# jackyko1991/vnet-tensorflow

Measured on AMD Instinct MI355X. Metric: training patches/sec (128^3x1ch fp32), higher is better.
Workload: dtype f32

## Files before the change

vnet_tensorflow_amd/csrc/conv_x3.h:

```cpp
#pragma once
#include "conv_kernels.h"

namespace {

constexpr int X3_TZ = 2, X3_TY = 8, X3_TX = 16;
constexpr int X3_IZ = X3_TZ + 4, X3_IY = X3_TY + 4, X3_IX = X3_TX + 4;
constexpr int X3_NV = X3_IZ * X3_IY * X3_IX;

template <bool W8>
struct X3G {
    static constexpr int TZ = W8 ? 4 : 2;
    static constexpr int IZ = TZ + 4, IY = X3_IY, IX = W8 ? 12 : X3_IX;
    static constexpr int ROWB = IX * 16;
    static constexpr int ZB = IY * ROWB + (W8 ? 64 : 0);
    static constexpr int PLANEB = IZ * ZB;
    static constexpr int PIECEB = 2 * PLANEB;
    static constexpr int TILEB = 3 * PIECEB;
    static constexpr int LDS = TILEB + 2 * 8 * 32 * 4;
    static constexpr int SPER = W8 ? 8 : 12;
};
static_assert(X3G<false>::PLANEB == X3_NV * 16 && X3G<false>::PLANEB % 256 == 0 && X3G<true>::PLANEB % 256 == 0, "tile planes");
static_assert((2 * X3G<true>::ZB) % 256 == 128, "lanes 8..15 of the narrow brick: the other half of the 256-byte bank row");
constexpr int X3_LDS = X3G<false>::LDS;

template <int K, int N, typename F>
__device__ __forceinline__ void x3_for_impl(F&& f) {
    if constexpr (K < N) { f(std::integral_constant<int, K>{}); x3_for_impl<K + 1, N>(f); }
}
template <int N, typename F>
__device__ __forceinline__ void x3_for(F&& f) { x3_for_impl<0, N>(f); }

typedef const __attribute__((address_space(1))) u32x4* x3_gw_t;
template <int NP>
__device__ __forceinline__ void x3_load_a(bf16x8 (&A)[NP][3], const u32x4* __restrict__ wbase, unsigned u0, unsigned ustride, int lane) {
    x3_for<NP * 3>([&](auto I) {
        constexpr int p = decltype(I)::value / 3, s = decltype(I)::value % 3;
        A[p][s] = __builtin_bit_cast(bf16x8, *(x3_gw_t)(wbase + (u0 + (unsigned)p * ustride + (unsigned)s * 64u) + lane));
    });
}
__device__ __forceinline__ void x3_load_a1(bf16x8 (&A)[3], const u32x4* __restrict__ wbase, unsigned u0, int lane) {
    x3_for<3>([&](auto I) {
        constexpr int s = decltype(I)::value;
        A[s] = __builtin_bit_cast(bf16x8, *(x3_gw_t)(wbase + (u0 + (unsigned)s * 64u) + lane));
    });
}

template <typename G>
__device__ __forceinline__ void x3_read_b(bf16x8 (&B)[3], const unsigned char* p) {
    B[0] = *reinterpret_cast<const bf16x8*>(p);
    B[1] = *reinterpret_cast<const bf16x8*>(p + G::PIECEB);
    B[2] = *reinterpret_cast<const bf16x8*>(p + 2 * G::PIECEB);
}

#define X3_PROD_A(k) ((k) == 0 ? 2 : (k) == 1 ? 0 : (k) == 2 ? 1 : (k) == 3 ? 1 : (k) == 4 ? 0 : 0)
#define X3_PROD_B(k) ((k) == 0 ? 0 : (k) == 1 ? 2 : (k) == 2 ? 1 : (k) == 3 ? 0 : (k) == 4 ? 1 : 0)

template <typename G, int DY0, int NDY, int A0 = 0, int NA = NDY>
__device__ __forceinline__ void x3_zrows(f32x4 (&acc)[8], const unsigned char* bz, const bf16x8 (&A)[NA][3]) {
    constexpr int J0 = DY0, J1 = DY0 + NDY + 7;
    bf16x8 Bn[3];
    x3_read_b<G>(Bn, bz + J0 * G::ROWB);
    x3_for<J1 - J0>([&](auto JI) {
        constexpr int jr = J0 + decltype(JI)::value;
        bf16x8 B[3] = {Bn[0], Bn[1], Bn[2]};
        if constexpr (jr + 1 < J1) x3_read_b<G>(Bn, bz + (jr + 1) * G::ROWB);
        __builtin_amdgcn_sched_barrier(0);
        x3_for<6 * NDY>([&](auto KI) {
            constexpr int k = decltype(KI)::value / NDY, d = decltype(KI)::value % NDY, m = jr - DY0 - d;
            if constexpr (m >= 0 && m < 8)
                acc[m] = __builtin_amdgcn_mfma_f32_16x16x32_bf16(A[A0 + d][X3_PROD_A(k)], B[X3_PROD_B(k)], acc[m], 0, 0, 0);
        });
        __builtin_amdgcn_sched_barrier(0);
    });
}

template <typename G, int A0, int NA>
__device__ __forceinline__ void x3_yrows_pairs(f32x4 (&acc)[8], const unsigned char* by, const bf16x8 (&A)[NA][3]) {
    bf16x8 Bn[3];
    x3_read_b<G>(Bn, by);
    x3_for<10>([&](auto KI) {
        constexpr int k = decltype(KI)::value;
        bf16x8 B[3] = {Bn[0], Bn[1], Bn[2]};
        if constexpr (k + 1 < 10) x3_read_b<G>(Bn, by + (k + 1) * G::ROWB);
        __builtin_amdgcn_sched_barrier(0);
        x3_for<6>([&](auto TI) {
            constexpr int t = decltype(TI)::value;
            if constexpr (k < 8) acc[k] = __builtin_amdgcn_mfma_f32_16x16x32_bf16(A[A0][X3_PROD_A(t)], B[X3_PROD_B(t)], acc[k], 0, 0, 0);
            if constexpr (k >= 2) acc[k - 2] = __builtin_amdgcn_mfma_f32_16x16x32_bf16(A[A0 + 1][X3_PROD_A(t)], B[X3_PROD_B(t)], acc[k - 2], 0, 0, 0);
        });
        __builtin_amdgcn_sched_barrier(0);
    });
}
template <typename G, int A0, int NA>
__device__ __forceinline__ void x3_yrows_single(f32x4 (&acc)[8], const unsigned char* b0, const bf16x8 (&A)[NA][3]) {
    bf16x8 Bn[3];
    x3_read_b<G>(Bn, b0 + 4 * G::ROWB);
    x3_for<8>([&](auto MI) {
        constexpr int m = decltype(MI)::value;
        bf16x8 B[3] = {Bn[0], Bn[1], Bn[2]};
        if constexpr (m + 1 < 8) x3_read_b<G>(Bn, b0 + (m + 5) * G::ROWB);
        __builtin_amdgcn_sched_barrier(0);
        x3_for<6>([&](auto TI) {
            constexpr int t = decltype(TI)::value;
            acc[m] = __builtin_amdgcn_mfma_f32_16x16x32_bf16(A[A0][X3_PROD_A(t)], B[X3_PROD_B(t)], acc[m], 0, 0, 0);
        });
        __builtin_amdgcn_sched_barrier(0);
    });
}

template <bool STATS, int NB, bool W8 = false>
__global__ void __launch_bounds__(512) __attribute__((amdgpu_waves_per_eu(2, 2))) conv5_x3_kernel(ConvArgs a) {
    constexpr int NT = 512;
    using G = X3G<W8>;
    using XT = XTile<X3_IZ, X3_IY, X3_IX, NT>;
    static_assert(XT::PER * XT::RPI == XT::ROWS && XT::PER == X3G<false>::SPER, "every staging pass covers whole tile rows");
    extern __shared__ __attribute__((aligned(16))) unsigned char smem[];
    unsigned char* tile = smem;
    float* red = reinterpret_cast<float*>(smem);
    float* sred = reinterpret_cast<float*>(smem + G::TILEB);
    const int tid = threadIdx.x;
    const int lane = tid & 63, wave = __builtin_amdgcn_readfirstlane(tid >> 6);
    const int j = lane & 15, g = lane >> 4, half = g & 1, hi = g >> 1;
    const int grp = wave >> 2, kw = wave & 3;

    const int base0 = W8 ? half * G::PLANEB + (grp + 2 * (j >> 3)) * G::ZB + (j & 7) * 16
                         : half * G::PLANEB + ((grp * G::IY) * G::IX + j) * 16;
    const unsigned char* bZ = tile + base0 + hi * G::ZB;
    const unsigned char* bY = tile + base0 + hi * G::ROWB + 4 * G::ZB;
    const unsigned char* b0 = tile + base0 + 4 * G::ZB;
    const unsigned char* bX = b0 + hi * 16;

    const int ncob = a.CoutP >> 4, ncobg = ncob / NB;
    const int nbrick = a.B * a.nbz * a.nby * a.nbx;
    const int nks = a.nz;
    const int nitems = nbrick * ncobg * nks;
    const int G8 = gridDim.x >> 3;
    const int per_xcd = (nitems + 7) >> 3;
    const int xcd = blockIdx.x & 7, slot = blockIdx.x >> 3;
    const int i_lo = xcd * per_xcd, i_hi = min(nitems, i_lo + per_xcd);
    if (i_lo + slot >= i_hi) return;
    const int nmine = (i_hi - i_lo - slot + G8 - 1) / G8;
    const int nch = a.cps;
    const int nsteps = nmine * nch;
    const unsigned astride = (unsigned)ncob * 3u * 64u;
    const u32x4* wbase = reinterpret_cast<const u32x4*>(a.wp);

    auto item_coords = [&](int it, int& b, int& bz, int& by, int& bx, int& cob) {
        int item = (i_lo + slot + it * G8) / nks;
        cob = (item % ncobg) * NB; item /= ncobg;
        bx = item % a.nbx; item /= a.nbx;
        by = item % a.nby; item /= a.nby;
        bz = item % a.nbz; b = item / a.nbz;
    };
    typedef const __attribute__((address_space(1))) f32x4* gf4_t;
    f32x4 pv[G::SPER];
    const int stid = W8 ? (tid < 384 ? tid : tid - 128) : (tid < XT::RPI * XT::COLS ? tid : tid - XT::COLS);
    constexpr int SCOLS = W8 ? 32 : XT::COLS;
    const int sr0 = stid / SCOLS, scol = stid - sr0 * SCOLS;
    const int six = scol >> 2, scq = scol & 3;
    auto tile_issue = [&](int step) {
        const int it = step / nch, ch = ((i_lo + slot + it * G8) % nks) * nch + (step - it * nch);
        int b, bz, by, bx, cob;
        item_coords(it, b, bz, by, bx, cob);
        const int c0 = ch * 16;
        const bool first = c0 < a.C0;
        const int cs = first ? a.C0 : a.C1;
        const float* src = (first ? a.x0 + c0 : a.x1 + (c0 - a.C0)) + (size_t)b * a.Di * a.Hi * a.Wi * cs;
        if constexpr (W8) {
            const int gz0 = bz * G::TZ - 2, gy = by * X3_TY - 2 + sr0;
            const bool yok = (unsigned)gy < (unsigned)a.Hi;
            const int rs = a.Wi * cs;
            const int off0 = (gy * a.Wi + six) * cs + scq * 4;
            x3_for<G::SPER>([&](auto KI) {
                constexpr int k = decltype(KI)::value;
                const int gz = gz0 + k;
                const bool ok = yok && (unsigned)gz < (unsigned)a.Di;
                const int off = off0 + gz * a.Hi * rs;
                gf4_t p = ok ? (gf4_t)(src + off) : (gf4_t)(vnet_zero_line);
                pv[k] = *p;
            });
        } else {
            const int gz0 = bz * X3_TZ - 2, gy = by * X3_TY - 2 + sr0, gx = bx * X3_TX - 2 + six;
            const bool xok = (unsigned)gx < (unsigned)a.Wi;
            const bool yok0 = xok && (unsigned)gy < (unsigned)a.Hi, yok1 = xok && (unsigned)(gy + 6) < (unsigned)a.Hi;
            const int rs = a.Wi * cs;
            const int off0 = (gy * a.Wi + gx) * cs + scq * 4;
            x3_for<XT::PER>([&](auto KI) {
                constexpr int k = decltype(KI)::value;
                const int gz = gz0 + (k >> 1);
                const bool ok = ((k & 1) ? yok1 : yok0) && (unsigned)gz < (unsigned)a.Di;
                const int off = off0 + gz * a.Hi * rs + (k & 1) * 6 * rs;
                gf4_t p = ok ? (gf4_t)(src + off) : (gf4_t)(vnet_zero_line);
                pv[k] = *p;
            });
        }
    };
    const unsigned cbase = (unsigned)((scq >> 1) * G::PLANEB + (six + (W8 ? 2 : 0)) * 16 + (scq & 1) * 8 + sr0 * G::ROWB);
    auto tile_commit = [&](const unsigned sgn) {
        unsigned cb = cbase;
        asm volatile("" : "+v"(cb));
        unsigned char* base = tile + cb;
        x3_for<G::SPER>([&](auto KI) {
            constexpr int k = decltype(KI)::value;
            u32x2 h, m, l;
            x3_split4(make_float4(__uint_as_float(__float_as_uint(pv[k][0]) ^ sgn), __uint_as_float(__float_as_uint(pv[k][1]) ^ sgn),
                                  __uint_as_float(__float_as_uint(pv[k][2]) ^ sgn), __uint_as_float(__float_as_uint(pv[k][3]) ^ sgn)), h, m, l);
            unsigned char* dst = base + k * (W8 ? G::ZB : XT::RPI * G::ROWB);
            *reinterpret_cast<u32x2*>(dst) = h;
            *reinterpret_cast<u32x2*>(dst + G::PIECEB) = m;
            *reinterpret_cast<u32x2*>(dst + 2 * G::PIECEB) = l;
        });
    };
    auto zero_halo = [&]() {
        if constexpr (W8) {
            int t0 = tid;
            asm volatile("" : "+v"(t0));
#pragma unroll 1
            for (int q = t0; q < 3 * 2 * 96 * 4; q += NT) {
                const int c = q & 3, row = (q >> 2) % 96, ph = q / (96 * 4);
                const int iz = row / 12, iy = row - iz * 12;
                *reinterpret_cast<u32x4*>(tile + ph * G::PLANEB + iz * G::ZB + iy * G::ROWB + (c < 2 ? c : c + 8) * 16) = u32x4{0u, 0u, 0u, 0u};
            }
        }
    };
    zero_halo();
    tile_issue(0);
    tile_commit(0u);
    __syncthreads();

    f32x4 acc[NB][8];
    VNET_STAMP_DECL;
    for (int step = 0; step < nsteps; ++step) {
        VNET_STAMP_STEP(step);
        VNET_STAMP(0);
        const int it = step / nch, lc = step - it * nch, ks = (i_lo + slot + it * G8) % nks, ch = ks * nch + lc;
        const bool first = lc == 0, last = lc == nch - 1, more = step + 1 < nsteps;
        int b, bz, by, bx, cob;
        item_coords(it, b, bz, by, bx, cob);
        if (first) x3_for<8 * NB>([&](auto MI) { acc[decltype(MI)::value / 8][decltype(MI)::value % 8] = f32x4{0.f, 0.f, 0.f, 0.f}; });
        else x3_for<8 * NB>([&](auto MI) { acc[decltype(MI)::value / 8][decltype(MI)::value % 8] = -acc[decltype(MI)::value / 8][decltype(MI)::value % 8]; });
        const int kc = (kw + ch) & 3;
        x3_for<NB>([&](auto NBI) {
            constexpr int nb = decltype(NBI)::value;
            const unsigned wc = (unsigned)(ch * X3_NPAIR * ncob + cob + nb) * 3u * 64u;
            bf16x8 A[5][3];
            if (grp) __builtin_amdgcn_s_setprio(1); else __builtin_amdgcn_s_setprio(0);
            x3_load_a<5>(A, wbase, wc + (unsigned)(kc * 5) * astride, astride, lane);
            __builtin_amdgcn_sched_barrier(0);
            x3_zrows<G, 0, 5>(acc[nb], bZ + kc * 16, A);
            __builtin_amdgcn_sched_barrier(0);
            if constexpr (nb == 0) VNET_STAMP(1);
            x3_load_a<5>(A, wbase, wc + (unsigned)(25 + kc * 5) * astride, astride, lane);
            __builtin_amdgcn_sched_barrier(0);
            x3_zrows<G, 0, 5>(acc[nb], bZ + 2 * G::ZB + kc * 16, A);
            __builtin_amdgcn_sched_barrier(0);
            if constexpr (nb == 0) VNET_STAMP(2);
            x3_load_a1(A[0], wbase, wc + (unsigned)(50 + kc * 2) * astride, lane);
            x3_load_a1(A[1], wbase, wc + (unsigned)(51 + kc * 2) * astride, lane);
            x3_load_a1(A[2], wbase, wc + (unsigned)(60 + (kc & 1)) * astride, lane);
            x3_load_a1(A[3], wbase, wc + 62u * astride, lane);
            __builtin_amdgcn_sched_barrier(0);
            if (grp) __builtin_amdgcn_s_setprio(0); else __builtin_amdgcn_s_setprio(1);
            if constexpr (nb == NB - 1) tile_issue(min(step + 1, nsteps - 1));
            __builtin_amdgcn_sched_barrier(0);
            x3_yrows_pairs<G, 0, 5>(acc[nb], bY + kc * 16, A);
            if (kc < 2) x3_yrows_single<G, 2, 5>(acc[nb], bX + kc * 32, A);
            if (kc == 3) x3_yrows_single<G, 3, 5>(acc[nb], b0 + 4 * 16, A);
            __builtin_amdgcn_sched_barrier(0);
            if constexpr (nb == 0) VNET_STAMP(3);
            {
                const int p0 = kc == 0 ? 20 : kc == 1 ? 23 : kc == 2 ? 46 : 49;
                const int p1 = kc == 0 ? 21 : kc == 1 ? 24 : kc == 2 ? 47 : 58;
                const int p2 = kc == 0 ? 22 : kc == 1 ? 45 : kc == 2 ? 48 : 59;
                x3_load_a1(A[0], wbase, wc + (unsigned)p0 * astride, lane);
                x3_load_a1(A[1], wbase, wc + (unsigned)p1 * astride, lane);
                x3_load_a1(A[2], wbase, wc + (unsigned)p2 * astride, lane);
            }
            __builtin_amdgcn_sched_barrier(0);
            if (kc == 0) {
                x3_zrows<G, 0, 3, 0, 5>(acc[nb], bZ + 4 * 16, A);
            } else if (kc == 1) {
                x3_zrows<G, 3, 2, 0, 5>(acc[nb], bZ + 4 * 16, A);
                x3_zrows<G, 0, 1, 2, 5>(acc[nb], bZ + 2 * G::ZB + 4 * 16, A);
            } else if (kc == 2) {
                x3_zrows<G, 1, 3, 0, 5>(acc[nb], bZ + 2 * G::ZB + 4 * 16, A);
            } else {
                x3_zrows<G, 4, 1, 0, 5>(acc[nb], bZ + 2 * G::ZB + 4 * 16, A);
                x3_yrows_pairs<G, 1, 5>(acc[nb], bY + 4 * 16, A);
            }
            __builtin_amdgcn_sched_barrier(0);
        });
        VNET_STAMP(4);
        __builtin_amdgcn_s_setprio(0);
        __syncthreads();
        VNET_STAMP(5);
        if (last) {
            const bool flip = lc & 1;
            x3_for<8 * NB>([&](auto MI) {
                constexpr int nb = decltype(MI)::value / 8, m = decltype(MI)::value % 8;
                *reinterpret_cast<f32x4*>(red + (((wave * NB + nb) * 8 + m) * 64 + lane) * 4) = flip ? -acc[nb][m] : acc[nb][m];
            });
            __syncthreads();
            x3_for<NB>([&](auto NBI) {
            constexpr int nb = decltype(NBI)::value;
            const int co0 = (cob + nb) * 16, co = co0 + 4 * g;
            f32x4 o[2];
            x3_for<2>([&](auto TI) {
                constexpr int t = decltype(TI)::value;
                const int m = 2 * kw + t;
                constexpr int WS = NB * 8 * 64 * 4;
                const float* rp = red + (((grp * 4 * NB + nb) * 8 + m) * 64 + lane) * 4;
                o[t] = (*reinterpret_cast<const f32x4*>(rp) + *reinterpret_cast<const f32x4*>(rp + WS)) +
                       (*reinterpret_cast<const f32x4*>(rp + 2 * WS) + *reinterpret_cast<const f32x4*>(rp + 3 * WS));
            });
            float bias4[4] = {0.f, 0.f, 0.f, 0.f};
            if (a.bias && co < a.Cout) {
                const float4 bb = *reinterpret_cast<const float4*>(a.bias + co);
                bias4[0] = bb.x; bias4[1] = bb.y; bias4[2] = bb.z; bias4[3] = bb.w;
            }
            float s1[4] = {0.f, 0.f, 0.f, 0.f}, s2[4] = {0.f, 0.f, 0.f, 0.f};
            const int oz = W8 ? bz * G::TZ + grp + 2 * (j >> 3) : bz * X3_TZ + grp, ox = W8 ? (j & 7) : bx * X3_TX + j;
            x3_for<2>([&](auto TI) {
                constexpr int t = decltype(TI)::value;
                const int oy = by * X3_TY + 2 * kw + t;
                if (oz < a.Do && oy < a.Ho && ox < a.Wo && co < a.Cout) {
                    const size_t ov = ((size_t)(b * a.Do + oz) * a.Ho + oy) * a.Wo + ox;
                    if (a.part) {
                        *reinterpret_cast<f32x4*>(a.part + (size_t)ks * a.part_stride + ov * a.CoutP + co) = o[t];
                        return;
                    }
                    float e[4] = {o[t][0] + bias4[0], o[t][1] + bias4[1], o[t][2] + bias4[2], o[t][3] + bias4[3]};
                    if constexpr (STATS) {
                        float4 rr = make_float4(0.f, 0.f, 0.f, 0.f);
                        if (a.res) rr = *reinterpret_cast<const float4*>(a.res + ov * a.Cout + co);
                        const float vv[4] = {e[0] + rr.x, e[1] + rr.y, e[2] + rr.z, e[3] + rr.w};
                        s1[0] += vv[0]; s1[1] += vv[1]; s1[2] += vv[2]; s1[3] += vv[3];
                        s2[0] += vv[0] * vv[0]; s2[1] += vv[1] * vv[1]; s2[2] += vv[2] * vv[2]; s2[3] += vv[3] * vv[3];
                    }
                    float* p = (co < a.Cy0) ? a.y0 + ov * a.Cy0 + co : a.y1 + ov * a.Cy1 + (co - a.Cy0);
                    if (a.accum) {
                        const float4 old = *reinterpret_cast<const float4*>(a.accsrc ? a.accsrc + ov * a.Cy0 + co : p);
                        e[0] += old.x; e[1] += old.y; e[2] += old.z; e[3] += old.w;
                    }
                    *reinterpret_cast<float4*>(p) = make_float4(e[0], e[1], e[2], e[3]);
                }
            });
            if constexpr (STATS) {
                x3_for<4>([&](auto KI) {
                    constexpr int k = decltype(KI)::value;
                    s1[k] = row16_sum(s1[k]); s2[k] = row16_sum(s2[k]);
                    if (j == 0) { sred[(nb * 8 + wave) * 32 + 4 * g + k] = s1[k]; sred[(nb * 8 + wave) * 32 + 16 + 4 * g + k] = s2[k]; }
                });
            }
            });
            __syncthreads();
            if constexpr (STATS) {
                int brick = (i_lo + slot + it * G8) / (ncobg * nks);
                x3_for<NB>([&](auto NBI) {
                    constexpr int nb = decltype(NBI)::value;
                    stats_row_write<8, 16>(sred + nb * 8 * 32, a.stats, (size_t)brick, (cob + nb) * 16, a.Cout, tid);
                });
            }
        }
        VNET_STAMP(6);
        if (last) zero_halo();
        if (more) tile_commit(((last ? 0 : lc + 1) & 1) ? 0x80000000u : 0u);
        VNET_STAMP(7);
        __syncthreads();
        VNET_STAMP(8);
        VNET_STAMP_FLUSH(step, wave, lane, 9);
    }
}

template <bool W8>
struct XWG {
    static constexpr int TZ = W8 ? 4 : 2;
    static constexpr int IZ = TZ + 4, IX = W8 ? 12 : X3_IX;
    static constexpr int XROW = IX * 32, XPLANE = X3_IY * XROW;
    static constexpr int XPB = IZ * XPLANE;
    static constexpr int DPB = 2 * X3_TY * 16 * 32;
    static constexpr int LDS = 3 * XPB + 3 * DPB;
    static constexpr int XHALF = W8 ? 2 * XPLANE : 8 * 32;
    static constexpr int XPER = W8 ? 8 : 12;
};
static_assert(XWG<false>::XROW % 256 == 128 && XWG<true>::XROW % 256 == 128, "row pairs of a k-step on disjoint banks");
constexpr int XW_LDS = XWG<false>::LDS;

__device__ __forceinline__ void xw_frag(bf16x8 (&F)[3], const unsigned char* lo, const unsigned char* hi, int pieceb) {
    typedef s16x4 __attribute__((address_space(3))) * lp;
#pragma unroll
    for (int s = 0; s < 3; ++s) {
        const s16x4 a = __builtin_amdgcn_ds_read_tr16_b64_v4i16((lp)(lo + s * pieceb));
        const s16x4 b = __builtin_amdgcn_ds_read_tr16_b64_v4i16((lp)(hi + s * pieceb));
        const s16x8 v = {a[0], a[1], a[2], a[3], b[0], b[1], b[2], b[3]};
        F[s] = __builtin_bit_cast(bf16x8, v);
    }
}

__device__ __forceinline__ void xw_mfma6(f32x4& acc, const bf16x8 (&A)[3], const bf16x8 (&B)[3]) {
#pragma unroll
    for (int k = 0; k < 6; ++k) acc = __builtin_amdgcn_mfma_f32_16x16x32_bf16(A[X3_PROD_A(k)], B[X3_PROD_B(k)], acc, 0, 0, 0);
}

template <bool W8>
__global__ void __launch_bounds__(512) __attribute__((amdgpu_waves_per_eu(2, 2))) wgrad5_x3_kernel(WgradArgs a) {
    constexpr int NT = 512;
    using G = XWG<W8>;
    constexpr int XW_XPB = G::XPB, XW_DPB = G::DPB, XW_XROW = G::XROW, XW_XPLANE = G::XPLANE;
    using XT = XTile<X3_IZ, X3_IY, X3_IX, NT>;
    static_assert(XT::PER == XWG<false>::XPER, "staging passes of the wide brick");
    extern __shared__ __attribute__((aligned(16))) unsigned char smem[];
    unsigned char* xt = smem;
    unsigned char* dyt = smem + 3 * XW_XPB;
    const int tid = threadIdx.x;
    const int lane = tid & 63, wave = __builtin_amdgcn_readfirstlane(tid >> 6);
    const int i = lane & 15, g = lane >> 4;
    const int split = blockIdx.x;
    const int chunk = blockIdx.y / a.ncob, cob = blockIdx.y - chunk * a.ncob;
    const int co0 = cob * 16;

    const int lane_x = W8 ? ((g & 1) * G::IX + (i >> 2)) * 32 + (g >> 1) * G::XHALF + (i & 3) * 8
                            : (((g & 1) * X3_IX + (g >> 1) * 8) + (i >> 2)) * 32 + (i & 3) * 8;
    const unsigned char* pb[3];
#pragma unroll
    for (int c = 0; c < 3; ++c) {
        const int q = 3 * wave + c, dz = q / 5, dx = q - dz * 5;
        pb[c] = xt + dz * XW_XPLANE + dx * 32 + lane_x;
    }
    const bool extra = wave < 5;
    const unsigned char* pe = xt + 4 * XW_XPLANE + (extra ? wave : 0) * XW_XROW + 4 * 32 + lane_x;
    const int lane_d = (((g & 1) * 16 + (g >> 1) * 8) + (i >> 2)) * 32 + (i & 3) * 8;
    const unsigned char* pa_lo = dyt + lane_d + (g & 1) * 128;
    const unsigned char* pa_hi = dyt + lane_d + (1 - (g & 1)) * 128;

    f32x4 acc[16];
#pragma unroll
    for (int t = 0; t < 16; ++t) acc[t] = f32x4{0.f, 0.f, 0.f, 0.f};

    float4 px[G::XPER], pd[2];
    auto brick_coords = [&](int brick, int& b, int& bz, int& by, int& bx) {
        bx = brick % a.nbx; brick /= a.nbx;
        by = brick % a.nby; brick /= a.nby;
        bz = brick % a.nbz; b = brick / a.nbz;
    };
    auto issue = [&](int brick) {
        int b, bz, by, bx;
        brick_coords(brick, b, bz, by, bx);
        if constexpr (W8) {
            const int stid = tid < 384 ? tid : tid - 128;
            const int iy = stid >> 5, col = stid & 31;
            const int c = chunk * 16 + (col & 3) * 4;
            const bool first = c < a.C0;
            const int cs = first ? a.C0 : a.C1;
            const float* src = (first ? a.x0 + c : a.x1 + (c - a.C0)) + (size_t)b * a.Di * a.Hi * a.Wi * cs;
            const int gz0 = bz * G::TZ - 2, gy = by * X3_TY - 2 + iy;
            const bool yok = (unsigned)gy < (unsigned)a.Hi;
            const int rs = a.Wi * cs, off0 = (gy * a.Wi + (col >> 2)) * cs;
#pragma unroll
            for (int k = 0; k < G::XPER; ++k) {
                const int gz = gz0 + k;
                const bool ok = yok && (unsigned)gz < (unsigned)a.Di;
                const float4 t = *reinterpret_cast<const float4*>(src + (ok ? off0 + gz * a.Hi * rs : 0));
                px[k] = ok ? t : make_float4(0.f, 0.f, 0.f, 0.f);
            }
        } else {
            XT::template issue_part<0, XT::PER>(px, a.x0, a.x1, a.C0, a.C1, chunk, b, bz * X3_TZ - 2, by * X3_TY - 2, bx * X3_TX - 2, a.Di, a.Hi, a.Wi, tid);
        }
#pragma unroll
        for (int k = 0; k < 2; ++k) {
            const int q = tid + k * NT;
            const int v = q >> 2, cq = q & 3;
            const int vx = v & 15, vy = (v >> 4) & 7, vz = v >> 7;
            const int oz = W8 ? bz * G::TZ + vz + 2 * (vx >> 3) : bz * X3_TZ + vz, oy = by * X3_TY + vy, ox = W8 ? (vx & 7) : bx * X3_TX + vx;
            const int c = co0 + cq * 4;
            const bool ok = oz < a.Do && oy < a.Ho && ox < a.Wo && c < a.Cout;
            const size_t ov = ok ? ((size_t)(b * a.Do + oz) * a.Ho + oy) * a.Wo + ox : 0;
            const float4 t = *reinterpret_cast<const float4*>(a.dy + ov * a.Cout + (ok ? c : 0));
            pd[k] = ok ? t : make_float4(0.f, 0.f, 0.f, 0.f);
        }
    };
    auto commit = [&](const bool neg) {
        if constexpr (W8) {
            const int stid = tid < 384 ? tid : tid - 128;
            unsigned char* base = xt + (stid >> 5) * XW_XROW + (((stid & 31) >> 2) + 2) * 32 + (stid & 3) * 8;
#pragma unroll
            for (int k = 0; k < G::XPER; ++k) {
                u32x2 h, m, l;
                x3_split4(px[k], h, m, l);
                unsigned char* dst = base + k * XW_XPLANE;
                *reinterpret_cast<u32x2*>(dst) = h;
                *reinterpret_cast<u32x2*>(dst + XW_XPB) = m;
                *reinterpret_cast<u32x2*>(dst + 2 * XW_XPB) = l;
            }
        } else {
        const int r0 = tid / XT::COLS, col = tid - r0 * XT::COLS;
        if (r0 < XT::RPI) {
            unsigned char* base = xt + (col >> 2) * 32 + (col & 3) * 8;
#pragma unroll
            for (int k = 0; k < XT::PER; ++k) {
                const int row = r0 + k * XT::RPI;
                u32x2 h, m, l;
                x3_split4(px[k], h, m, l);
                unsigned char* dst = base + row * XW_XROW;
                *reinterpret_cast<u32x2*>(dst) = h;
                *reinterpret_cast<u32x2*>(dst + XW_XPB) = m;
                *reinterpret_cast<u32x2*>(dst + 2 * XW_XPB) = l;
            }
        }
        }
#pragma unroll
        for (int k = 0; k < 2; ++k) {
            const int q = tid + k * NT;
            const int v = q >> 2, cq = q & 3;
            const int vx = v & 15, row = v >> 4;
            u32x2 h, m, l;
            const float4 dv = neg ? make_float4(-pd[k].x, -pd[k].y, -pd[k].z, -pd[k].w) : pd[k];
            x3_split4(dv, h, m, l);
            unsigned char* dst = dyt + (row * 16 + (vx ^ ((row & 1) << 2))) * 32 + cq * 8;
            *reinterpret_cast<u32x2*>(dst) = h;
            *reinterpret_cast<u32x2*>(dst + XW_DPB) = m;
            *reinterpret_cast<u32x2*>(dst + 2 * XW_DPB) = l;
        }
    };

    bool neg = false;
    if constexpr (W8) {
        for (int q = tid; q < 3 * G::IZ * X3_IY * 4 * 2; q += NT) {
            const int hf = q & 1, c = (q >> 1) & 3, row = (q >> 3) % (G::IZ * X3_IY), piece = q / (8 * G::IZ * X3_IY);
            *reinterpret_cast<u32x4*>(xt + piece * XW_XPB + row * XW_XROW + (c < 2 ? c : c + 8) * 32 + hf * 16) = u32x4{0u, 0u, 0u, 0u};
        }
    }
    if (split < a.nbrick) issue(split);
    for (int brick = split; brick < a.nbrick; brick += a.nsplit) {
        __syncthreads();
        commit(neg);
        __syncthreads();
        if (brick != split) {
#pragma unroll
            for (int t = 0; t < 16; ++t) acc[t] = -acc[t];
        }
        neg = !neg;
        auto plane = [&](const int zz) {
            if ((wave >> 2) ^ zz) __builtin_amdgcn_s_setprio(1); else __builtin_amdgcn_s_setprio(0);
            const int zx = zz * XW_XPLANE, zd = zz * (X3_TY * 16 * 32);
#pragma unroll
            for (int c = 0; c < 3; ++c) {
                const unsigned char* p = pb[c] + zx;
                bf16x8 F[5][3], A[3], An[3];
#pragma unroll
                for (int r = 0; r < 5; ++r) xw_frag(F[r], p + r * XW_XROW, p + r * XW_XROW + 128, XW_XPB);
                xw_frag(An, pa_lo + zd, pa_hi + zd, XW_DPB);
#pragma unroll
                for (int s = 0; s < 4; ++s) {
#pragma unroll
                    for (int q = 0; q < 3; ++q) A[q] = An[q];
                    if (s + 1 < 4) xw_frag(An, pa_lo + zd + (s + 1) * 1024, pa_hi + zd + (s + 1) * 1024, XW_DPB);
                    __builtin_amdgcn_sched_barrier(0);
                    xw_mfma6(acc[c * 5 + 0], A, F[(2 * s + 0) % 5]);
                    xw_mfma6(acc[c * 5 + 1], A, F[(2 * s + 1) % 5]);
                    __builtin_amdgcn_sched_barrier(0);
                    if (s + 1 < 4) {
                        xw_frag(F[(2 * s + 0) % 5], p + (2 * s + 5) * XW_XROW, p + (2 * s + 5) * XW_XROW + 128, XW_XPB);
                        xw_frag(F[(2 * s + 1) % 5], p + (2 * s + 6) * XW_XROW, p + (2 * s + 6) * XW_XROW + 128, XW_XPB);
                    }
                    __builtin_amdgcn_sched_barrier(0);
                    xw_mfma6(acc[c * 5 + 2], A, F[(2 * s + 2) % 5]);
                    xw_mfma6(acc[c * 5 + 3], A, F[(2 * s + 3) % 5]);
                    xw_mfma6(acc[c * 5 + 4], A, F[(2 * s + 4) % 5]);
                    __builtin_amdgcn_sched_barrier(0);
                }
            }
            if (extra) {
                const unsigned char* p = pe + zx;
                bf16x8 E[3], En[3], A[3], An[3];
                xw_frag(En, p, p + 128, XW_XPB);
                xw_frag(An, pa_lo + zd, pa_hi + zd, XW_DPB);
#pragma unroll
                for (int s = 0; s < 4; ++s) {
#pragma unroll
                    for (int q = 0; q < 3; ++q) { A[q] = An[q]; E[q] = En[q]; }
                    if (s + 1 < 4) {
                        xw_frag(An, pa_lo + zd + (s + 1) * 1024, pa_hi + zd + (s + 1) * 1024, XW_DPB);
                        xw_frag(En, p + (2 * s + 2) * XW_XROW, p + (2 * s + 2) * XW_XROW + 128, XW_XPB);
                    }
                    __builtin_amdgcn_sched_barrier(0);
                    xw_mfma6(acc[15], A, E);
                    __builtin_amdgcn_sched_barrier(0);
                }
            }
        };
        plane(0);
        __builtin_amdgcn_sched_barrier(0);
        issue(brick + a.nsplit < a.nbrick ? brick + a.nsplit : brick);
        __builtin_amdgcn_sched_barrier(0);
        plane(1);
    }
    __builtin_amdgcn_s_setprio(0);
    if (!neg) {
#pragma unroll
        for (int t = 0; t < 16; ++t) acc[t] = -acc[t];
    }
#pragma unroll
    for (int t = 0; t < 16; ++t) {
        int tap;
        if (t < 15) { const int q = 3 * wave + t / 5, dz = q / 5, dx = q - dz * 5; tap = (dz * 5 + t % 5) * 5 + dx; }
        else { if (!extra) continue; tap = (4 * 5 + wave) * 5 + 4; }
        float* dst = a.part + ((size_t)(split * 125 + tap) * a.CinP + chunk * 16 + i) * a.CoutP + co0 + g * 4;
        const f32x4 r = acc[t];
        *reinterpret_cast<float4*>(dst) = make_float4(r.x, r.y, r.z, r.w);
    }
}

inline int x3_conv_nbz(int D, int W) { return W == 8 ? ceil_div(D, X3G<true>::TZ) : ceil_div(D, X3_TZ); }
inline int x3_conv_bricks(int B, int D, int H, int W) { return B * x3_conv_nbz(D, W) * ceil_div(H, X3_TY) * ceil_div(W, X3_TX); }
struct X3WgradPlan { int nbz, nby, nbx, nbrick, nsplit, nblk; };
inline X3WgradPlan x3_plan_wgrad(int Cin, int Cout, int B, int D, int H, int W) {
    X3WgradPlan p{};
    p.nbz = x3_conv_nbz(D, W); p.nby = ceil_div(H, X3_TY); p.nbx = ceil_div(W, X3_TX);
    p.nbrick = B * p.nbz * p.nby * p.nbx;
    p.nblk = (Cin / 16) * (Cout / 16);
    p.nsplit = max(1, min(p.nbrick, ceil_div(256, p.nblk)));
    return p;
}
inline bool x3_wgrad_ok(int C0, int C1, int Cout, int B, int D, int H, int W) {
    if (C0 <= 0 || Cout <= 0 || (C0 & 15) || (C1 & 15) || (Cout & 15) || (W < 16 && W != 8)) return false;
    const X3WgradPlan p = x3_plan_wgrad(C0 + C1, Cout, B, D, H, W);
    return p.nbrick >= (W == 8 ? 2 : 4) * p.nsplit;
}

struct X3Plan { int ok, nks, cps; long items; };
inline X3Plan x3_plan_conv(int C0, int C1, int Cy0, int Cy1, int B, int D, int H, int W) {
    X3Plan p{0, 1, 0, 0};
    if (C0 <= 0 || Cy0 <= 0 || (C0 & 15) || (C1 & 15) || (Cy0 & 15) || (Cy1 & 15) || (W < 16 && W != 8)) return p;
    const int nch = (C0 + C1) / 16;
    p.items = (long)x3_conv_bricks(B, D, H, W) * ((Cy0 + Cy1) / 16);
    p.cps = nch;
    while (p.items * p.nks < 256 && p.cps % 2 == 0 && p.cps >= 4) { p.nks *= 2; p.cps /= 2; }
    p.ok = p.items * p.nks >= 192;
    return p;
}
inline bool x3_conv_ok(int C0, int C1, int Cy0, int Cy1, int B, int D, int H, int W) { return x3_plan_conv(C0, C1, Cy0, Cy1, B, D, H, W).ok != 0; }

}
```

Measured before the change: 69.44.

## Split NB=2 conv work so each wave group owns one output block and reuses weights across z-planes

For NB=2, the two wave groups no longer both cover both output-channel blocks. Each group now loads weights for its own channel block and applies each loaded weight fragment to two z-plane offsets from the shared tile. This halves the weight (A) loads per MFMA and reuses register-resident weights across spatial positions. The reduction slot mapping is changed to match the new ownership. The W8 variant is excluded, and the new accumulator layout must map correctly onto the epilogue reduction.

```diff
diff --git a/vnet_tensorflow_amd/csrc/conv_x3.h b/vnet_tensorflow_amd/csrc/conv_x3.h
--- a/vnet_tensorflow_amd/csrc/conv_x3.h
+++ b/vnet_tensorflow_amd/csrc/conv_x3.h
@@ -123,8 +123,9 @@
     const int j = lane & 15, g = lane >> 4, half = g & 1, hi = g >> 1;
     const int grp = wave >> 2, kw = wave & 3;
 
+    static_assert(NB == 1 || !W8, "the block split is built for the wide brick");
     const int base0 = W8 ? half * G::PLANEB + (grp + 2 * (j >> 3)) * G::ZB + (j & 7) * 16
-                         : half * G::PLANEB + ((grp * G::IY) * G::IX + j) * 16;
+                         : half * G::PLANEB + (((NB == 2 ? 0 : grp) * G::IY) * G::IX + j) * 16;
     const unsigned char* bZ = tile + base0 + hi * G::ZB;
     const unsigned char* bY = tile + base0 + hi * G::ROWB + 4 * G::ZB;
     const unsigned char* b0 = tile + base0 + 4 * G::ZB;
@@ -240,34 +241,42 @@
         if (first) x3_for<8 * NB>([&](auto MI) { acc[decltype(MI)::value / 8][decltype(MI)::value % 8] = f32x4{0.f, 0.f, 0.f, 0.f}; });
         else x3_for<8 * NB>([&](auto MI) { acc[decltype(MI)::value / 8][decltype(MI)::value % 8] = -acc[decltype(MI)::value / 8][decltype(MI)::value % 8]; });
         const int kc = (kw + ch) & 3;
-        x3_for<NB>([&](auto NBI) {
-            constexpr int nb = decltype(NBI)::value;
-            const unsigned wc = (unsigned)(ch * X3_NPAIR * ncob + cob + nb) * 3u * 64u;
+        {
+            const unsigned wc = (unsigned)(ch * X3_NPAIR * ncob + cob + (NB == 2 ? grp : 0)) * 3u * 64u;
             bf16x8 A[5][3];
             if (grp) __builtin_amdgcn_s_setprio(1); else __builtin_amdgcn_s_setprio(0);
             x3_load_a<5>(A, wbase, wc + (unsigned)(kc * 5) * astride, astride, lane);
             __builtin_amdgcn_sched_barrier(0);
-            x3_zrows<G, 0, 5>(acc[nb], bZ + kc * 16, A);
-            __builtin_amdgcn_sched_barrier(0);
-            if constexpr (nb == 0) VNET_STAMP(1);
+            x3_for<NB>([&](auto PI) {
+                constexpr int p = decltype(PI)::value, po = p * G::ZB;
+                x3_zrows<G, 0, 5>(acc[p], bZ + po + kc * 16, A);
+                __builtin_amdgcn_sched_barrier(0);
+            });
+            VNET_STAMP(1);
             x3_load_a<5>(A, wbase, wc + (unsigned)(25 + kc * 5) * astride, astride, lane);
             __builtin_amdgcn_sched_barrier(0);
-            x3_zrows<G, 0, 5>(acc[nb], bZ + 2 * G::ZB + kc * 16, A);
-            __builtin_amdgcn_sched_barrier(0);
-            if constexpr (nb == 0) VNET_STAMP(2);
+            x3_for<NB>([&](auto PI) {
+                constexpr int p = decltype(PI)::value, po = p * G::ZB;
+                x3_zrows<G, 0, 5>(acc[p], bZ + po + 2 * G::ZB + kc * 16, A);
+                __builtin_amdgcn_sched_barrier(0);
+            });
+            VNET_STAMP(2);
             x3_load_a1(A[0], wbase, wc + (unsigned)(50 + kc * 2) * astride, lane);
             x3_load_a1(A[1], wbase, wc + (unsigned)(51 + kc * 2) * astride, lane);
             x3_load_a1(A[2], wbase, wc + (unsigned)(60 + (kc & 1)) * astride, lane);
             x3_load_a1(A[3], wbase, wc + 62u * astride, lane);
             __builtin_amdgcn_sched_barrier(0);
             if (grp) __builtin_amdgcn_s_setprio(0); else __builtin_amdgcn_s_setprio(1);
-            if constexpr (nb == NB - 1) tile_issue(min(step + 1, nsteps - 1));
+            tile_issue(min(step + 1, nsteps - 1));
             __builtin_amdgcn_sched_barrier(0);
-            x3_yrows_pairs<G, 0, 5>(acc[nb], bY + kc * 16, A);
-            if (kc < 2) x3_yrows_single<G, 2, 5>(acc[nb], bX + kc * 32, A);
-            if (kc == 3) x3_yrows_single<G, 3, 5>(acc[nb], b0 + 4 * 16, A);
-            __builtin_amdgcn_sched_barrier(0);
-            if constexpr (nb == 0) VNET_STAMP(3);
+            x3_for<NB>([&](auto PI) {
+                constexpr int p = decltype(PI)::value, po = p * G::ZB;
+                x3_yrows_pairs<G, 0, 5>(acc[p], bY + po + kc * 16, A);
+                if (kc < 2) x3_yrows_single<G, 2, 5>(acc[p], bX + po + kc * 32, A);
+                if (kc == 3) x3_yrows_single<G, 3, 5>(acc[p], b0 + po + 4 * 16, A);
+                __builtin_amdgcn_sched_barrier(0);
+            });
+            VNET_STAMP(3);
             {
                 const int p0 = kc == 0 ? 20 : kc == 1 ? 23 : kc == 2 ? 46 : 49;
                 const int p1 = kc == 0 ? 21 : kc == 1 ? 24 : kc == 2 ? 47 : 58;
@@ -277,19 +286,22 @@
                 x3_load_a1(A[2], wbase, wc + (unsigned)p2 * astride, lane);
             }
             __builtin_amdgcn_sched_barrier(0);
-            if (kc == 0) {
-                x3_zrows<G, 0, 3, 0, 5>(acc[nb], bZ + 4 * 16, A);
-            } else if (kc == 1) {
-                x3_zrows<G, 3, 2, 0, 5>(acc[nb], bZ + 4 * 16, A);
-                x3_zrows<G, 0, 1, 2, 5>(acc[nb], bZ + 2 * G::ZB + 4 * 16, A);
-            } else if (kc == 2) {
-                x3_zrows<G, 1, 3, 0, 5>(acc[nb], bZ + 2 * G::ZB + 4 * 16, A);
-            } else {
-                x3_zrows<G, 4, 1, 0, 5>(acc[nb], bZ + 2 * G::ZB + 4 * 16, A);
-                x3_yrows_pairs<G, 1, 5>(acc[nb], bY + 4 * 16, A);
-            }
-            __builtin_amdgcn_sched_barrier(0);
-        });
+            x3_for<NB>([&](auto PI) {
+                constexpr int p = decltype(PI)::value, po = p * G::ZB;
+                if (kc == 0) {
+                    x3_zrows<G, 0, 3, 0, 5>(acc[p], bZ + po + 4 * 16, A);
+                } else if (kc == 1) {
+                    x3_zrows<G, 3, 2, 0, 5>(acc[p], bZ + po + 4 * 16, A);
+                    x3_zrows<G, 0, 1, 2, 5>(acc[p], bZ + po + 2 * G::ZB + 4 * 16, A);
+                } else if (kc == 2) {
+                    x3_zrows<G, 1, 3, 0, 5>(acc[p], bZ + po + 2 * G::ZB + 4 * 16, A);
+                } else {
+                    x3_zrows<G, 4, 1, 0, 5>(acc[p], bZ + po + 2 * G::ZB + 4 * 16, A);
+                    x3_yrows_pairs<G, 1, 5>(acc[p], bY + po + 4 * 16, A);
+                }
+                __builtin_amdgcn_sched_barrier(0);
+            });
+        }
         VNET_STAMP(4);
         __builtin_amdgcn_s_setprio(0);
         __syncthreads();
@@ -298,7 +310,8 @@
             const bool flip = lc & 1;
             x3_for<8 * NB>([&](auto MI) {
                 constexpr int nb = decltype(MI)::value / 8, m = decltype(MI)::value % 8;
-                *reinterpret_cast<f32x4*>(red + (((wave * NB + nb) * 8 + m) * 64 + lane) * 4) = flip ? -acc[nb][m] : acc[nb][m];
+                const int slot = NB == 2 ? (nb * 4 + kw) * NB + grp : wave;
+                *reinterpret_cast<f32x4*>(red + ((slot * 8 + m) * 64 + lane) * 4) = flip ? -acc[nb][m] : acc[nb][m];
             });
             __syncthreads();
             x3_for<NB>([&](auto NBI) {
```

Measured after the change: 70.47, median of 6. 1.5% higher.
